# hiroyasuakada/EgoRear

Hardware: AMD Instinct MI355X
Metric: 4-view frames/sec (heatmap+MVFEx+3D lift) (higher is better)
Workload: dtype f32 (fp16x2 split, 22-bit operands, fp32 accumulate)

## Files before the change

### egorear_amd/csrc/egr_conv_chain.hip

```cpp
#include "egr_conv_shared.h"

using namespace egrc;

namespace {

#ifndef CHAIN_SB_G
#define CHAIN_SB_G 1
#endif
#ifndef CHAIN_SB_E
#define CHAIN_SB_E 1
#endif
#define SB_G() do { if (CHAIN_SB_G) __builtin_amdgcn_sched_barrier(0); } while (0)
#define SB_E() do { if (CHAIN_SB_E) __builtin_amdgcn_sched_barrier(0); } while (0)

struct ChainArgs {
    ConvArgs a;
    const void* w2;
    const float* wds2;
    const float* shift1;
    int64_t gw2, gp1;
    int act1;
};

constexpr int OOB = (int)0x80000000;

template <int KS1, int RESK>
__global__ __launch_bounds__(512) void conv_pw_chain_kernel(const ChainArgs ca) {
    constexpr int NCF = 4, KS2 = 8, NPL = 2;
    constexpr bool PIPE = true;
    constexpr int W1B = NCF * KS1 * NPL * 1024, W2B = NCF * KS2 * NPL * 1024;
    constexpr int PR = 16, PATCH = PR * 144;
    constexpr int VEC = 4 * 128 * 4;
    static_assert(W1B + W2B + VEC + 8 * PATCH <= 160 * 1024, "LDS");
    __shared__ __attribute__((aligned(16))) uint8_t lds[W1B + W2B + VEC + 8 * PATCH];
    float* const s_sc1 = reinterpret_cast<float*>(lds + W1B + W2B);
    float* const s_sh1 = s_sc1 + 128;
    float* const s_sc2 = s_sh1 + 128;
    float* const s_sh2 = s_sc2 + 128;
    const ConvArgs& a = ca.a;
    const egr_conv_desc& d = a.d;
    const int grp = blockIdx.z;
    const int tid = threadIdx.x, lane = tid & 63, wave = tid >> 6, p = lane & 31, h = lane >> 5;
    float sa, ads;
    act_prescale(a.amax_in, lane, sa, ads);
    float amx = 0.f;
    unsigned lb0 = lane * 16, lb1 = lane * 16 + 65536;
    asm volatile("" : "+v"(lb0), "+v"(lb1));
    auto wfrag = [&](const int off) __attribute__((always_inline)) {
        return off < 65536 ? *reinterpret_cast<const u32x4*>(lds + lb0 + off) : *reinterpret_cast<const u32x4*>(lds + lb1 + (off - 65536));
    };
    const __amdgpu_buffer_rsrc_t rx = __builtin_amdgcn_make_buffer_rsrc(uniform_ptr(a.x + grp * d.gx), 0, 0x80000000u, 0x00020000);
    const __amdgpu_buffer_rsrc_t ry = __builtin_amdgcn_make_buffer_rsrc(uniform_ptr(a.y + grp * d.gy), 0, 0x80000000u, 0x00020000);
    const __amdgpu_buffer_rsrc_t rr = __builtin_amdgcn_make_buffer_rsrc(uniform_ptr(a.res ? a.res + grp * d.gr : a.x), 0, 0x80000000u, 0x00020000);
    const int HoWo = d.ho * d.wo;
    const int T = (a.M + 31) >> 5, NW = gridDim.x * 8;
    int t = blockIdx.x * 8 + wave;

    auto x_off = [&](int tile) {
        const int m = tile * 32 + p;
        int n, pix;
        if (a.howo_shift >= 0) { n = m >> a.howo_shift; pix = m & (HoWo - 1); }
        else { n = fdiv(m, a.dHoWo); pix = m - n * HoWo; }
        const int xb = a.x_plain ? n * (int)d.xmap.stride_inner : (int)fmap(d.xmap, a.dXin, n);
        return (tile < T && m < a.M) ? (xb + pix * d.ldx) * 4 + h * 16 : OOB;
    };
    u32x4 raw[2 * KS1];
    {
        typedef unsigned u32x2 __attribute__((ext_vector_type(2)));
        auto stage = [&](const uint8_t* img, auto ks_tag, uint8_t* dst0) __attribute__((always_inline)) {
            constexpr int KS = decltype(ks_tag)::value;
            constexpr int NV = NCF * KS * NPL * 64 / 512;
            u32x4 wv[NV];
#pragma unroll
            for (int i = 0; i < NV; ++i) {
                const int v = tid + 512 * i;
                const int cf = v / (KS * 64 * NPL), rem = v - cf * (KS * 64 * NPL);
                wv[i] = *reinterpret_cast<const u32x4*>(img + ((int64_t)cf * (KS / 2) * 2 * NPL) * 1024 + rem * 16);
            }
#pragma unroll
            for (int i = 0; i < NV; ++i) {
                const int v = tid + 512 * i;
                const int lo = v & 63, blk = v >> 6;
                uint8_t* const dst = dst0 + blk * 1024 + (lo & 31) * 16 + (lo >> 5) * 8;
                *reinterpret_cast<u32x2*>(dst) = u32x2{wv[i][0], wv[i][1]};
                *reinterpret_cast<u32x2*>(dst + 512) = u32x2{wv[i][2], wv[i][3]};
            }
        };
        const int xo = x_off(t);
#pragma unroll
        for (int i = 0; i < 2 * KS1; ++i) raw[i] = __builtin_amdgcn_raw_buffer_load_b128(rx, xo + i * 32, 0, 0);
        stage(reinterpret_cast<const uint8_t*>(a.w) + (int64_t)grp * d.gw * 2, std::integral_constant<int, KS1>{}, lds);
        stage(reinterpret_cast<const uint8_t*>(ca.w2) + (int64_t)grp * ca.gw2 * 2, std::integral_constant<int, KS2>{}, lds + W1B);
        if (tid < 128) {
            s_sc1[tid] = ads * a.wds[grp * ca.gp1 + tid];
            s_sh1[tid] = ca.shift1 ? ca.shift1[grp * ca.gp1 + tid] : 0.f;
            s_sc2[tid] = (tid < d.cout) ? ca.wds2[grp * d.gp + tid] * ((a.scale && tid < d.cout) ? a.scale[grp * d.gp + tid] : 1.f) : 1.f;
            s_sh2[tid] = (a.shift && tid < d.cout) ? a.shift[grp * d.gp + tid] : 0.f;
        }
    }
    __syncthreads();

    const float floor1 = (ca.act1 == EGR_ACT_RELU) ? 0.f : -__builtin_inff();
    const float floor_ = (d.act == EGR_ACT_RELU) ? 0.f : -__builtin_inff();
    const bool res_before = d.res_mode == EGR_RES_BEFORE_ACT;
    constexpr int PW[3] = {1, 0, 0}, PX[3] = {0, 1, 0};
    for (; t < T; t += NW) {
#ifdef CHAIN_EXP_NOLOAD
        const int xo_n = OOB;
#else
        const int xo_n = x_off(t + NW);
#endif
        f32x16 acc1[NCF];
// ... 53 lines not shown
                const f32x4 sc = *reinterpret_cast<const f32x4*>(s_sc1 + cf * 32 + 8 * g + 4 * h);
                const f32x4 sh = *reinterpret_cast<const f32x4*>(s_sh1 + cf * 32 + 8 * g + 4 * h);
#pragma unroll
                for (int e = 0; e < 4; ++e) {
                    float v = acc1[cf][4 * g + e] * sc[e] + sh[e];
                    v = v > floor1 ? v : floor1;
                    acc1[cf][4 * g + e] = v;
                    pmax = fmaxf(pmax, fabsf(v));
                }
            }
        pmax = fmaxf(pmax, __shfl_xor(pmax, 32, 64));
        int k2 = 141 - (int)(__float_as_uint(pmax) >> 23);
        k2 = k2 > 60 ? 60 : (k2 < -60 ? -60 : k2);
        const float sa2 = __uint_as_float((unsigned)(127 + k2) << 23), inv2 = __uint_as_float((unsigned)(127 - k2) << 23);
        SB_G();
        f32x16 acc2[NCF];
#pragma unroll
        for (int cf = 0; cf < NCF; ++cf)
#pragma unroll
            for (int r = 0; r < 16; ++r) acc2[cf][r] = 0.f;
        constexpr int S0 = KS1 & 1;
#pragma unroll
        for (int ks = 0; ks < KS2; ++ks) {
            const int cf1 = ks >> 1, g0 = 2 * (ks & 1);
            unsigned xh[4], xl[4];
#pragma unroll
            for (int e = 0; e < 4; ++e) {
                const int r0 = 4 * (g0 + (e >> 1)) + 2 * (e & 1);
                split2_f16(acc1[cf1][r0], acc1[cf1][r0 + 1], sa2, xh[e], xl[e]);
            }
            u32x4 xb[NPL];
            xb[0] = u32x4{xh[0], xh[1], xh[2], xh[3]};
            xb[1] = u32x4{xl[0], xl[1], xl[2], xl[3]};
            if constexpr (PIPE) {
                if (ks + 1 < KS2) read_w2((S0 + ks + 1) & 1, ks + 1);
            } else {
                read_w2(0, ks);
            }
            SB_G();
#pragma unroll
            for (int t3 = 0; t3 < 3; ++t3)
#pragma unroll
                for (int cf = 0; cf < NCF; ++cf)
#ifdef CHAIN_EXP_NOMFMA2
                    if (t3 == 0 && ks == 0)
#endif
                    acc2[cf] = mfma_split<NPL>(wf[PIPE ? ((S0 + ks) & 1) : 0][cf][PW[t3]], xb[PX[t3]], acc2[cf]);
            SB_G();
        }
        SB_G();
#pragma unroll
        for (int i = 0; i < 2 * KS1; ++i) raw[i] = __builtin_amdgcn_raw_buffer_load_b128(rx, xo_n + i * 32, 0, 0);
        SB_G();
        const int m = t * 32 + p;
        int n, pix;
        if (a.howo_shift >= 0) { n = m >> a.howo_shift; pix = m & (HoWo - 1); }
        else { n = fdiv(m, a.dHoWo); pix = m - n * HoWo; }
        const bool live = m < a.M;
        const int yo_p = live ? ((a.y_plain ? n * (int)d.ymap.stride_inner : (int)fmap(d.ymap, a.dYin, n)) + pix * d.ldy) * 4 : OOB;
        int ro_p = OOB, ox_p = 0, oy_p = 0;
        float lx1_p = 0.f, ly1_p = 0.f;
        if constexpr (RESK == 1) {
            if (live) ro_p = ((a.r_plain ? n * (int)d.rmap.stride_inner : (int)fmap(d.rmap, a.dRin, n)) + pix * d.ldr) * 4;
        }
        if constexpr (RESK == 2) {
            const int ho = (a.wo_shift >= 0) ? (pix >> a.wo_shift) : fdiv(pix, a.dWo), wo = pix - ho * d.wo;
            const int hl = d.ho >> 1, wl = d.wo >> 1;
            const float shh = (d.ho > 1) ? (float)(hl - 1) / (float)(d.ho - 1) : 0.f;
            const float sww = (d.wo > 1) ? (float)(wl - 1) / (float)(d.wo - 1) : 0.f;
            const float fy = shh * (float)ho, fx = sww * (float)wo;
            const int y0 = (int)fy, x0 = (int)fx;
            ly1_p = fminf(fmaxf(__builtin_fmaf(shh, (float)ho, -(float)y0), 0.f), 1.f);
            lx1_p = fminf(fmaxf(__builtin_fmaf(sww, (float)wo, -(float)x0), 0.f), 1.f);
            if (live) ro_p = ((a.r_plain ? n * (int)d.rmap.stride_inner : (int)fmap(d.rmap, a.dRin, n)) + (y0 * wl + x0) * d.ldr) * 4;
            ox_p = (x0 + 1 > wl - 1) ? 0 : d.ldr * 4;
            oy_p = (y0 + 1 > hl - 1) ? 0 : wl * d.ldr * 4;
        }
        const int qd = lane & 7, rsub = lane >> 3;
        uint8_t* const patch = lds + W1B + W2B + VEC + wave * PATCH;
        int yo[2][2], ro[2][2], ox[2][2], oy[2][2];
        float lx1[2][2], ly1[2][2];
#pragma unroll
        for (int hp = 0; hp < 2; ++hp)
#pragma unroll
            for (int i = 0; i < 2; ++i) {
                const int src = hp * 16 + i * 8 + rsub;
                yo[hp][i] = __shfl(yo_p, src) + qd * 16;
                if constexpr (RESK != 0) ro[hp][i] = __shfl(ro_p, src) + qd * 16;
                if constexpr (RESK == 2) {
                    ox[hp][i] = __shfl(ox_p, src); oy[hp][i] = __shfl(oy_p, src);
                    lx1[hp][i] = __shfl(lx1_p, src); ly1[hp][i] = __shfl(ly1_p, src);
                }
            }
        constexpr int NR = RESK == 2 ? 4 : (RESK == 1 ? 1 : 0);
        f32x4 rq[2][NR > 0 ? NR : 1];
        auto res_issue = [&](const int st, const int par) __attribute__((always_inline)) {
            if constexpr (RESK != 0) {
                const int hp = st >> 3, cf = (st >> 1) & 3, i = st & 1;
#ifdef CHAIN_EXP_NORES
                if (st > 0) return;
#endif
                const int r0 = (RESK == 1 && cf * 32 + 4 * qd >= d.cout) ? OOB : ro[hp][i] + cf * 128;
                rq[par][0] = __builtin_bit_cast(f32x4, __builtin_amdgcn_raw_buffer_load_b128(rr, r0, 0, 0));
                if constexpr (RESK == 2) {
                    rq[par][1] = __builtin_bit_cast(f32x4, __builtin_amdgcn_raw_buffer_load_b128(rr, ro[hp][i] + ox[hp][i] + cf * 128, 0, 0));
                    rq[par][2] = __builtin_bit_cast(f32x4, __builtin_amdgcn_raw_buffer_load_b128(rr, ro[hp][i] + oy[hp][i] + cf * 128, 0, 0));
                    rq[par][3] = __builtin_bit_cast(f32x4, __builtin_amdgcn_raw_buffer_load_b128(rr, ro[hp][i] + oy[hp][i] + ox[hp][i] + cf * 128, 0, 0));
// ... 307 lines not shown
        const bool live = t < T && m < a.M;
        const int yo_p = live ? ((a.y_plain ? n * (int)d.ymap.stride_inner : (int)fmap(d.ymap, a.dYin, n)) + pix * d.ldy) * 4 : OOB;
        const int qd = lane & 7, rsub = lane >> 3;
        uint8_t* const patch = lds + R * CH + VEC + wave * PATCH;
        int yo[2][2];
#pragma unroll
        for (int hp = 0; hp < 2; ++hp)
#pragma unroll
            for (int i = 0; i < 2; ++i) yo[hp][i] = __shfl(yo_p, hp * 16 + i * 8 + rsub) + qd * 16;
        auto patch_write = [&](const int u) __attribute__((always_inline)) {
            const int hp = u >> 2, cf = u & 3;
            if ((p >> 4) == hp) {
#pragma unroll
                for (int g = 0; g < 4; ++g)
                    *reinterpret_cast<f32x4*>(patch + (p & 15) * 144 + g * 32 + h * 16) =
                        f32x4{acc2[cf][4 * g] * inv2, acc2[cf][4 * g + 1] * inv2, acc2[cf][4 * g + 2] * inv2, acc2[cf][4 * g + 3] * inv2};
            }
        };
        patch_write(0);
#pragma unroll
        for (int u = 0; u < 8; ++u) {
            const int hp = u >> 2, cf = u & 3;
            __builtin_amdgcn_wave_barrier();
            f32x4 vv[2];
#pragma unroll
            for (int i = 0; i < 2; ++i) vv[i] = *reinterpret_cast<const f32x4*>(patch + (i * 8 + rsub) * 144 + qd * 16);
            const int c = cf * 32 + 4 * qd;
            const f32x4 sc = *reinterpret_cast<const f32x4*>(s_sc2 + c), sh = *reinterpret_cast<const f32x4*>(s_sh2 + c);
            const bool cok = c < d.cout;
            asm volatile("s_waitcnt lgkmcnt(0)" ::: "memory");
            __builtin_amdgcn_wave_barrier();
            if (u + 1 < 8) patch_write(u + 1);
#pragma unroll
            for (int i = 0; i < 2; ++i) {
                f32x4 v = vv[i];
#pragma unroll
                for (int e = 0; e < 4; ++e) {
                    float tt = v[e] * sc[e] + sh[e];
                    tt = tt > floor_ ? tt : floor_;
                    v[e] = tt;
                }
                if (cok && yo[hp][i] >= 0) amx = fmaxf(fmaxf(amx, fmaxf(fabsf(v[0]), fabsf(v[1]))), fmaxf(fabsf(v[2]), fabsf(v[3])));
                __builtin_amdgcn_raw_buffer_store_b128(__builtin_bit_cast(u32x4, v), ry, cok ? yo[hp][i] + cf * 128 : OOB, 0, 0);
            }
        }
    }
    if (a.amax_out) amax_flush(a.amax_out, amx, (int)blockIdx.x * NWV + wave);
}

int g_chain_blocks = getenv("EGR_CONV_CHAIN_BLOCKS") ? atoi(getenv("EGR_CONV_CHAIN_BLOCKS")) : 256;

}

extern "C" int egr_conv1x1_chain_f32(const egr_conv_desc* dd, const float* x, const void* w1, const float* shift2, const float* res, float* y,
                                     const egr_conv_aux* aux, const egr_chain_aux* chain, void* stream) {
    if (!dd || !x || !w1 || !y || !aux || !chain || !aux->w_descale || !aux->amax_in || !chain->w2 || !chain->w2_descale) return EGR_ENULL;
    ChainArgs ca;
    ConvArgs& a = ca.a;
    a = ConvArgs{};
    a.d = *dd;
    egr_conv_desc& d = a.d;
    if (d.groups <= 0) d.groups = 1;
    if (d.kh != 1 || d.kw != 1 || d.stride != 1 || d.pad != 0 || d.h != d.ho || d.w != d.wo || d.transposed || d.out_nchw || d.split_k > 1) return EGR_EINVAL;
    const bool big = d.cin == 256 && chain->cmid == 256;
    if (!big && ((d.cin != 64 && d.cin != 128) || chain->cmid != 128)) return EGR_EINVAL;
    if (d.cout <= 0 || d.cout > 128 || d.cout % 4 != 0) return EGR_EINVAL;
    if (big && d.res_mode != EGR_RES_NONE) return EGR_EINVAL;
    if (d.w_format != EGR_W_F16X2 || d.n <= 0 || d.ho <= 0 || d.wo <= 0 || d.groups > 65535) return EGR_EINVAL;
    if ((d.act != EGR_ACT_NONE && d.act != EGR_ACT_RELU) || (chain->act1 != EGR_ACT_NONE && chain->act1 != EGR_ACT_RELU)) return EGR_EINVAL;
    if (d.res_mode != EGR_RES_NONE && !res) return EGR_ENULL;
    if (d.res_mode == EGR_RES_UP2_BEFORE_ACT && ((d.ho | d.wo) & 1)) return EGR_EINVAL;
    if (d.ldx % 4 != 0 || d.ldy % 4 != 0 || (d.res_mode && d.ldr % 4 != 0)) return EGR_EINVAL;
    if (((uintptr_t)x | (uintptr_t)w1 | (uintptr_t)chain->w2 | (uintptr_t)y | (uintptr_t)res) & 15) return EGR_EINVAL;
    if (((uintptr_t)aux->amax_in | (uintptr_t)aux->amax_out) & 3) return EGR_EINVAL;
    if (d.xmap.n_inner <= 0 || d.ymap.n_inner <= 0 || (d.res_mode && d.rmap.n_inner <= 0)) return EGR_EINVAL;
    if (((d.xmap.stride_inner | d.xmap.stride_outer | d.ymap.stride_inner | d.ymap.stride_outer) % 4) != 0) return EGR_EINVAL;
    if (d.res_mode && ((d.rmap.stride_inner | d.rmap.stride_outer) % 4) != 0) return EGR_EINVAL;
    if (d.groups > 1 && (((d.gx | d.gp | d.gy | d.gr | chain->gp1) % 4) != 0 || (d.gw | chain->gw2) % 8 != 0)) return EGR_EINVAL;
    const int64_t M64 = (int64_t)d.n * d.ho * d.wo;
    if (M64 >= (1LL << 31)) return EGR_EINVAL;
    auto span = [](const egr_nmap& m, int n) {
        const int o = (n - 1) / m.n_inner, i = (n - 1 < m.n_inner ? n - 1 : m.n_inner - 1);
        return (int64_t)i * m.stride_inner + (int64_t)o * m.stride_outer;
    };
    if ((span(d.xmap, d.n) + (int64_t)d.h * d.w * d.ldx) * 4 + 64 >= (1LL << 31)) return EGR_EINVAL;
    if ((span(d.ymap, d.n) + (int64_t)d.ho * d.wo * d.ldy) * 4 >= (1LL << 31)) return EGR_EINVAL;
    if (d.res_mode && (span(d.rmap, d.n) + (int64_t)d.ho * d.wo * d.ldr) * 4 >= (1LL << 31)) return EGR_EINVAL;
    a.x = x; a.w = static_cast<const float*>(w1); a.shift = shift2; a.res = res; a.y = y;
    a.wds = aux->w_descale; a.amax_in = aux->amax_in; a.amax_out = aux->amax_out;
    a.M = (int)M64;
    a.Npad = 128;
    a.K = d.cin;
    auto log2_exact = [](int v) { int l = 0; while ((1 << l) < v) ++l; return ((1 << l) == v) ? l : -1; };
    a.howo_shift = log2_exact(d.ho * d.wo);
    a.wo_shift = log2_exact(d.wo);
    a.x_plain = d.xmap.n_inner >= d.n;
    a.y_plain = d.ymap.n_inner >= d.n;
    a.r_plain = d.res_mode ? (d.rmap.n_inner >= d.n) : 1;
    a.dHoWo = make_fastdiv(d.ho * d.wo);
    a.dWo = make_fastdiv(d.wo);
    a.dXin = make_fastdiv(d.xmap.n_inner);
    a.dYin = make_fastdiv(d.ymap.n_inner);
    a.dRin = make_fastdiv(d.res_mode ? d.rmap.n_inner : 1);
    a.cblocks = d.cin / BK;
    a.taps = 1;
    a.ktiles = a.cblocks;
    ca.w2 = chain->w2; ca.wds2 = chain->w2_descale; ca.shift1 = chain->shift1; ca.gw2 = chain->gw2; ca.gp1 = chain->gp1; ca.act1 = chain->act1;
    int nblk = g_chain_blocks / d.groups;
    if (nblk < 1) nblk = 1;
    const int t32 = (a.M + 31) / 32;
    if (nblk * 8 > t32) nblk = (t32 + 7) / 8;
    const dim3 grid((unsigned)nblk, 1, (unsigned)d.groups);
    const int resk = d.res_mode == EGR_RES_NONE ? 0 : (d.res_mode == EGR_RES_UP2_BEFORE_ACT ? 2 : 1);
    hipStream_t s = (hipStream_t)stream;
    if (big) {
        static const int nwv = getenv("EGR_CONV_CHAIN_BIG_WAVES") ? atoi(getenv("EGR_CONV_CHAIN_BIG_WAVES")) : 8;
        if (nwv == 8) {
            hipLaunchKernelGGL((conv_pw2_kernel<0, 8>), grid, dim3(512), 0, s, ca);
        } else {
            int nb4 = 2 * g_chain_blocks / d.groups;
            if (nb4 < 1) nb4 = 1;
            if (nb4 * 4 > t32) nb4 = (t32 + 3) / 4;
            hipLaunchKernelGGL((conv_pw2_kernel<0, 4>), dim3((unsigned)nb4, 1, (unsigned)d.groups), dim3(256), 0, s, ca);
        }
        return egr_launch_status();
    }
    if (d.cin == 64) {
        if (resk == 0) hipLaunchKernelGGL((conv_pw_chain_kernel<4, 0>), grid, dim3(512), 0, s, ca);
        else if (resk == 1) hipLaunchKernelGGL((conv_pw_chain_kernel<4, 1>), grid, dim3(512), 0, s, ca);
        else hipLaunchKernelGGL((conv_pw_chain_kernel<4, 2>), grid, dim3(512), 0, s, ca);
    } else {
        if (resk == 0) hipLaunchKernelGGL((conv_pw_chain_kernel<8, 0>), grid, dim3(512), 0, s, ca);
        else if (resk == 1) hipLaunchKernelGGL((conv_pw_chain_kernel<8, 1>), grid, dim3(512), 0, s, ca);
        else hipLaunchKernelGGL((conv_pw_chain_kernel<8, 2>), grid, dim3(512), 0, s, ca);
    }
    return egr_launch_status();
}
```

### egorear_amd/hip.py

```python
from __future__ import annotations

import ctypes as C
import os
import threading
from typing import Optional, Union

import torch

_HERE = os.path.dirname(os.path.abspath(__file__))
LIB_PATH = os.environ.get("EGR_LIB") or os.path.join(_HERE, "csrc", "libegorear_hip.so")

ACT_NONE, ACT_RELU, ACT_GELU = 0, 1, 2
RES_NONE, RES_BEFORE_ACT, RES_AFTER_ACT, RES_UP2_BEFORE_ACT = 0, 1, 2, 3



import contextlib
import dataclasses
import sys
import types


class _on_default:

    def __init__(self, fn):
        self.fn = fn
        self.__doc__ = fn.__doc__

    def __get__(self, obj, cls):
        return types.MethodType(self.fn, obj if obj is not None else cls())


@dataclasses.dataclass
class LaunchPolicy:
    w_format: str = "f16x2"
    h2: bool = True
    x6_min_rows: int = 4096
    x6_min_flops: float = 5e8
    x6_train_min_rows: int = 8192
    x6_train_min_flops: float = 4e9
    chain: bool = True
    chain_min_rows: int = 8192
    chain_big: bool = True
    chain_big_min_rows: int = 65536
    wgrad_x6: bool = True
    wgrad_force: bool = False
    layer_h2: bool = True
    fused_layer: bool = True
    fused_query: bool = True
    train_one_product: bool = False

    @classmethod
    def from_env(cls, env=None) -> "LaunchPolicy":
        e = os.environ if env is None else env
        fmt = e.get("EGR_W_FORMAT", "f16x2")
        fp16 = fmt in ("f16x2", "f16")
        tfmt = e.get("EGR_TRAIN_FORMAT", "")
        if tfmt not in ("", "f16") or (tfmt == "f16" and fmt != "f16"):
            raise ValueError("egorear_amd: EGR_TRAIN_FORMAT=f16 is the only value, and it requires EGR_W_FORMAT=f16")
        return cls(train_one_product=tfmt == "f16", w_format=fmt, h2=fp16,
                   x6_min_rows=int(e.get("EGR_X6_MIN_ROWS", "4096")), x6_min_flops=float(e.get("EGR_X6_MIN_FLOPS", "5e8")),
                   x6_train_min_rows=int(e.get("EGR_X6_TRAIN_MIN_ROWS", "8192")), x6_train_min_flops=float(e.get("EGR_X6_TRAIN_MIN_FLOPS", "4e9")),
                   chain=e.get("EGR_CONV_CHAIN", "1") != "0", chain_min_rows=int(e.get("EGR_CONV_CHAIN_MIN_ROWS", "8192")),
                   chain_big=e.get("EGR_CONV_CHAIN_BIG", "1") != "0", chain_big_min_rows=int(e.get("EGR_CONV_CHAIN_BIG_MIN_ROWS", "65536")),
                   wgrad_x6=fmt != "f32", layer_h2=fp16 and e.get("EGR_LAYER_H2", "1") != "0",
                   fused_layer=e.get("EGR_FUSED_LAYER", "1") != "0", fused_query=e.get("EGR_FUSED_QUERY", "1") != "0")

    def replace(self, **kw) -> "LaunchPolicy":
        return dataclasses.replace(self, **kw)

    def pack_key(self) -> tuple:
        key = (self.w_format, self.h2, self.layer_h2)
        return key + ("train_f16",) if self.train_one_product else key

    def exact(self) -> "LaunchPolicy":
        return self.replace(w_format="bf16x3", h2=False, layer_h2=False)

    @_on_default
    def fast(self) -> "LaunchPolicy":
        return self.replace(w_format="f16", h2=True, layer_h2=True)

    @_on_default
    def fast_training(self) -> "LaunchPolicy":
        return self.fast().replace(train_one_product=True)

    @property
    def fp16_scheme(self) -> bool:
        return self.w_format in ("f16x2", "f16")


POLICY = LaunchPolicy.from_env()
_POLICY_TLS = threading.local()


def policy() -> LaunchPolicy:
    cur = getattr(_POLICY_TLS, "cur", None)
    return cur if cur is not None else POLICY


@contextlib.contextmanager
def use_policy(p: Optional[LaunchPolicy]):
    if p is None:
        yield
        return
    old = getattr(_POLICY_TLS, "cur", None)
    _POLICY_TLS.cur = p
    try:
        yield
    finally:
        _POLICY_TLS.cur = old


def install_policy_properties(module_name: str, mapping: dict) -> None:
    def make(field):
        return property(lambda self: getattr(policy(), field), lambda self, v: setattr(POLICY, field, v))
    mod = sys.modules[module_name]
    mod.__class__ = type("_PolicyModule", (types.ModuleType,), {name: make(field) for name, field in mapping.items()})


install_policy_properties(__name__, {
    "H2": "h2", "X6_MIN_ROWS": "x6_min_rows", "X6_MIN_FLOPS": "x6_min_flops", "X6_TRAIN_MIN_ROWS": "x6_train_min_rows",
    "X6_TRAIN_MIN_FLOPS": "x6_train_min_flops", "CHAIN": "chain", "CHAIN_MIN_ROWS": "chain_min_rows", "CHAIN_BIG": "chain_big",
    "CHAIN_BIG_MIN_ROWS": "chain_big_min_rows", "WGRAD_X6": "wgrad_x6", "WGRAD_FORCE": "wgrad_force"})

EXPORTS = [
    "egr_conv2d_nhwc_f32", "egr_stem_conv7x7_f32", "egr_maxpool_nhwc_f32", "egr_upsample2x_nhwc_f32",
    "egr_avgpool_nhwc_f32", "egr_argmax_rows_f32", "egr_layernorm_f32", "egr_joint_mha_f32", "egr_msda_gather_f32",
    "egr_fisheye_project_f32", "egr_linear_smallk_f32", "egr_jqa_sum_f32", "egr_tokens_to_nhwc_f32", "egr_version",
    "egr_device_arch", "egr_conv_force_config", "egr_preprocess_u8_f32", "egr_pose_metrics_f32", "egr_gt_heatmap_f32", "egr_conv_debug_stamps", "egr_conv2d_wgrad_f32", "egr_conv2d_masked_f32", "egr_up2_relu_head_f32",
    "egr_msda_fwd_f32", "egr_msda_bwd_f32", "egr_w6_elems", "egr_pack_w6_f32", "egr_pack_w6_many_f32", "egr_joint_layer_f32",
    "egr_preprocess_fused_u8_f32", "egr_preprocess_band_rows", "egr_conv_set_persist", "egr_stem_conv7x7_pool_f32",
    "egr_stem_w6_bytes", "egr_pack_stem_w6_f32", "egr_stem_conv7x7_x6_f32", "egr_wgrad_last_kernel", "egr_conv_last_kernel", "egr_conv_set_tap", "egr_conv_set_tapx", "egr_conv_set_splitk_fused", "egr_fisheye_project2_f32", "egr_pack_layer_w_f32", "egr_pack_layer_wh2_f32",
    "egr_conv2d_nhwc_ex_f32", "egr_wh2_elems", "egr_pack_wh2_f32", "egr_absmax_f32", "egr_stem_conv7x7_x6_ex_f32", "egr_stem_wh2_bytes", "egr_pack_stem_wh2_f32", "egr_stem_conv7x7_h2_f32",
    "egr_pack_wh2_many_f32", "egr_conv2d_masked_ex_f32", "egr_conv2d_wgrad_ex_f32", "egr_wgrad_last_h2", "egr_wgrad_last_planes",
    "egr_wstream_image_bytes", "egr_pack_wstream_f32", "egr_linear_wstream_workspace_bytes", "egr_linear_wstream_f32", "egr_conv1x1_chain_f32",
    "egr_jqa_query_f32", "egr_pose_query_f32", "egr_layer_set_planes", "egr_head_set_persist", "egr_heatmap_metrics_f32",
    "egr_conv_plan", "egr_soft_argmax_f32", "egr_soft_argmax_bwd_f32", "egr_coord_l1_f32",
    "egr_triangulate_f32", "egr_triangulate_bwd_f32", "egr_volume_fuse_f32", "egr_volume_fuse_bwd_f32",
    "egr_peaks_f32", "egr_consensus_f32",
]


class NMap(C.Structure):
    _fields_ = [("n_inner", C.c_int32), ("stride_inner", C.c_int64), ("stride_outer", C.c_int64)]


class ConvDesc(C.Structure):
    _fields_ = [
        ("n", C.c_int32), ("h", C.c_int32), ("w", C.c_int32), ("cin", C.c_int32), ("cout", C.c_int32),
        ("kh", C.c_int32), ("kw", C.c_int32), ("stride", C.c_int32), ("pad", C.c_int32),
        ("ho", C.c_int32), ("wo", C.c_int32), ("ldx", C.c_int32), ("ldy", C.c_int32), ("ldr", C.c_int32),
        ("xmap", NMap), ("ymap", NMap), ("rmap", NMap),
        ("act", C.c_int32), ("res_mode", C.c_int32), ("out_nchw", C.c_int32), ("split_k", C.c_int32),
        ("groups", C.c_int32),
        ("gx", C.c_int64), ("gw", C.c_int64), ("gp", C.c_int64), ("gy", C.c_int64), ("gr", C.c_int64),
        ("grs", C.c_int64), ("grm", C.c_int64),
        ("transposed", C.c_int32), ("w_format", C.c_int32),
    ]


class ConvAux(C.Structure):
    _fields_ = [("w_descale", C.c_void_p), ("amax_in", C.c_void_p), ("amax_out", C.c_void_p),
                ("bn_partials", C.c_void_p), ("bn_tiles_out", C.c_void_p), ("bn_capacity", C.c_int64)]


class ConvPlan(C.Structure):
    _fields_ = [(n, C.c_int32) for n in ("route", "bm", "bn", "variant", "planes", "tiles_m", "tiles_n", "grid_x", "grid_y", "grid_z", "block",
                                         "split_k", "ktiles_per_split", "persistent", "cls_mode", "fused_reduce", "reduce_pass", "bn_slabs")]


ROUTE_F32_TILED, ROUTE_SPLIT_TILED, ROUTE_TAP, ROUTE_TAP2, ROUTE_STREAM_1X1, ROUTE_SMALL_F32, ROUTE_TAPX = range(7)
W_F16X2, W_F16X1, W_F16X1T = 4, 8, 16


class ChainAux(C.Structure):
    _fields_ = [("w2", C.c_void_p), ("w2_descale", C.c_void_p), ("shift1", C.c_void_p), ("cmid", C.c_int32), ("act1", C.c_int32),
                ("gw2", C.c_int64), ("gp1", C.c_int64)]


class LayerDesc(C.Structure):
    _P = C.c_void_p
    _fields_ = ([(n, C.c_int32) for n in ("B", "J", "V", "C", "heads", "cf", "groups", "ffn_dim")] +
                [("eps", C.c_float), ("mha_scale", C.c_float)] +
                [(n, C.c_void_p) for n in ("x", "g", "e", "sigma", "rowmask",
                                           "w_fold", "c_fold", "w_out", "b_out", "w_fuse", "b_fuse", "ln1_g", "ln1_b",
                                           "w_qkv", "b_qkv", "w_mo", "b_mo", "ln2_g", "ln2_b", "w_f0", "b_f0", "w_f1", "b_f1", "ln3_g", "ln3_b",
                                           "x_out", "w_ol", "b_ol", "ol_out")] +
                [("ol_n", C.c_int32), ("w_packed", C.c_int32)] +
                [(n, C.c_void_p) for n in ("lnp_g", "lnp_b", "xn_out", "w_r0", "b_r0", "w_r2", "b_r2", "anchors3d", "pred_out",
                                           "w_h0", "b_h0", "h0_out", "amax_h0")] +
                [("h0_n", C.c_int32)])


class JqaQueryDesc(C.Structure):
    _fields_ = ([(n, C.c_int32) for n in ("B", "J", "C", "groups", "kb", "pool_hw", "ol_n", "w_packed")] +
                [(n, C.c_void_p) for n in ("t", "s32", "w_hp2", "b_hp2", "w_bfb", "b_bfb", "embed", "w_q", "b_q", "w_ol", "b_ol",
                                           "x_out", "ol_out")])


class PoseQueryDesc(C.Structure):
    _fields_ = ([(n, C.c_int32) for n in ("B", "J", "C", "ol_n", "w_packed")] +
                [(n, C.c_void_p) for n in ("h1", "w_m2", "b_m2", "ctm", "cams", "w_qg0", "b_qg0", "w_qg2", "b_qg2", "w_qg4", "b_qg4",
                                           "w_ol", "b_ol", "pred_out", "anchors3d_out", "anchors2d_out", "valid_out", "x_out", "ol_out")])


def _load() -> C.CDLL:
    if not os.path.exists(LIB_PATH):
        raise ImportError(
            f"{LIB_PATH} not found: build it with `python -m egorear_amd.csrc.build` "
            "(or __graft_entry__.build()).  egorear_amd has no CPU / PyTorch fallback.")
    lib = C.CDLL(LIB_PATH)
    vp, i32, i64, f32 = C.c_void_p, C.c_int32, C.c_int64, C.c_float
    lib.egr_conv2d_nhwc_f32.argtypes = [C.POINTER(ConvDesc), vp, vp, vp, vp, vp, vp, vp, vp, vp, C.c_size_t, vp]
    lib.egr_conv2d_nhwc_ex_f32.argtypes = [C.POINTER(ConvDesc), vp, vp, vp, vp, vp, vp, vp, vp, vp, C.c_size_t, C.POINTER(ConvAux), vp]
    lib.egr_conv_plan.argtypes = [C.POINTER(ConvDesc), vp, vp, vp, vp, vp, vp, vp, vp, vp, vp, C.c_size_t, C.POINTER(ConvAux), C.POINTER(ConvPlan)]
    lib.egr_conv1x1_chain_f32.argtypes = [C.POINTER(ConvDesc), vp, vp, vp, vp, vp, C.POINTER(ConvAux), C.POINTER(ChainAux), vp]
    lib.egr_fill_f32.argtypes = [vp, f32, i64, vp]
    lib.egr_fill_f32.restype = C.c_int
    lib.egr_absmax_f32.argtypes = [vp, i64, vp, vp]
    lib.egr_wh2_elems.restype = C.c_int64
    lib.egr_wh2_elems.argtypes = [i32, i32]
    lib.egr_pack_wh2_f32.argtypes = [vp, i32, i32, i32, vp, vp, vp]
    lib.egr_stem_conv7x7_f32.argtypes = [vp, NMap, i32, i32, i32, vp, vp, vp, vp, i32, i64, vp]
    lib.egr_stem_conv7x7_pool_f32.argtypes = [vp, NMap, i32, i32, i32, vp, vp, vp, vp, i32, i64, vp]
    lib.egr_wgrad_last_kernel.argtypes = []
    lib.egr_wgrad_last_planes.argtypes = []
    lib.egr_conv_last_kernel.argtypes = []
    lib.egr_conv_set_tap.argtypes = [i32]
    lib.egr_conv_set_tapx.argtypes = [i32, i32, i32]
    lib.egr_conv_set_splitk_fused.argtypes = [i32]
    lib.egr_stem_w6_bytes.restype = C.c_int64
    lib.egr_stem_w6_bytes.argtypes = []
    lib.egr_pack_stem_w6_f32.argtypes = [vp, i32, vp, vp]
    lib.egr_stem_conv7x7_x6_f32.argtypes = [vp, NMap, i32, i32, i32, vp, vp, vp, vp, i32, i32, i64, vp]
    lib.egr_stem_conv7x7_x6_ex_f32.argtypes = [vp, NMap, i32, i32, i32, vp, vp, vp, vp, i32, i32, i64, vp, vp]
    lib.egr_stem_wh2_bytes.restype = C.c_int64
    lib.egr_stem_wh2_bytes.argtypes = []
    lib.egr_pack_stem_wh2_f32.argtypes = [vp, i32, vp, vp, vp]
    lib.egr_stem_conv7x7_h2_f32.argtypes = [vp, NMap, i32, i32, i32, vp, vp, vp, vp, vp, i32, i32, i64, vp, vp]
    lib.egr_wstream_image_bytes.restype = C.c_int64
    lib.egr_wstream_image_bytes.argtypes = [i32, i32]
    lib.egr_pack_wstream_f32.argtypes = [vp, i32, i32, vp, vp, vp]
    lib.egr_linear_wstream_workspace_bytes.restype = C.c_int64
    lib.egr_linear_wstream_workspace_bytes.argtypes = [i32, i32, i32]
    lib.egr_linear_wstream_f32.argtypes = [vp, i64, i32, i32, vp, vp, vp, i32, i32, vp, vp, i64, vp, vp, i64, vp]
    lib.egr_maxpool_nhwc_f32.argtypes = [vp, vp, i32, i32, i32, i32, i32, i32, i32, vp]
    lib.egr_upsample2x_nhwc_f32.argtypes = [vp, i32, vp, i32, i32, i32, i32, i32, i32, vp]
    lib.egr_avgpool_nhwc_f32.argtypes = [vp, vp, i32, i32, i32, vp]
    lib.egr_argmax_rows_f32.argtypes = [vp, i32, i32, i32, f32, vp, vp, vp, vp, vp]
    lib.egr_soft_argmax_f32.argtypes = [vp, i32, i32, i32, f32, i32, i32, f32, vp, vp, vp, vp, vp, vp, vp]
    lib.egr_soft_argmax_bwd_f32.argtypes = [vp, vp, vp, vp, vp, vp, i32, i32, i32, f32, i32, i32, i32, vp, vp]
    lib.egr_triangulate_f32.argtypes = [vp, vp, vp, vp, i32, i32, i32, f32, f32, f32, f32, vp, vp, vp, vp, vp]
    lib.egr_triangulate_bwd_f32.argtypes = [vp, vp, vp, vp, i32, i32, i32, f32, f32, f32, f32, vp, vp, vp, vp, vp]
    lib.egr_volume_fuse_f32.argtypes = [vp, vp, vp, vp, vp, vp, i32, i32, i32, i32, i32, i32, f32, f32, f32, vp, vp, vp, vp, vp, vp]
    lib.egr_volume_fuse_bwd_f32.argtypes = [vp, vp, vp, vp, vp, vp, i32, i32, i32, i32, i32, i32, f32, f32, f32, vp, vp, vp, vp]
    lib.egr_peaks_f32.argtypes = [vp, i32, i32, i32, i32, i32, i32, f32, f32, vp, vp, vp, vp, vp]
    lib.egr_consensus_f32.argtypes = [vp, vp, vp, vp, vp, i32, i32, i32, i32, f32, f32, f32, i32, f32, vp, vp, vp, vp, vp, vp, vp]
    lib.egr_coord_l1_f32.argtypes = [vp, vp, vp, i32, i32, f32, vp, vp, vp]
    lib.egr_layernorm_f32.argtypes = [vp, vp, vp, vp, vp, i32, i32, f32, i32, vp]
    lib.egr_joint_mha_f32.argtypes = [vp, vp, i32, i32, i32, i32, f32, vp]
    lib.egr_msda_gather_f32.argtypes = [vp, i32, vp, i32, vp, vp, vp, i32, i32, i32, i32, i32, i32, vp, vp, vp, vp, i32, vp]
    lib.egr_fisheye_project_f32.argtypes = [vp, vp, vp, i32, i32, vp, vp, vp, vp]
    lib.egr_fisheye_project2_f32.argtypes = [vp, vp, vp, vp, i32, i32, vp, vp, vp, vp]
    lib.egr_linear_smallk_f32.argtypes = [vp, i64, i64, vp, vp, vp, i32, i32, i32, i32, i32, vp]
    lib.egr_jqa_sum_f32.argtypes = [vp, vp, vp, vp, i32, i32, i32, i32, vp]
    lib.egr_tokens_to_nhwc_f32.argtypes = [vp, vp, i32, i32, i32, vp]
    lib.egr_version.restype = C.c_char_p
    lib.egr_w6_elems.restype = C.c_int64
    lib.egr_device_arch.argtypes = [C.c_char_p, i32]
# ... 495 lines not shown
        return False
    return x.n * x.h * x.w >= (pol.chain_big_min_rows if big else pol.chain_min_rows)


def conv1x1_chain(x: Img, w1, w2, cmid: int, cout: int, *, shift1=None, shift2=None, act1: int = ACT_RELU, act2: int = ACT_NONE,
                  res: Optional[Img] = None, res_mode: int = RES_NONE, out: Optional[Img] = None, groups: int = 1,
                  amax_out: Optional[torch.Tensor] = None) -> Img:
    if not chain_eligible(x, w1, w2, cmid, cout, groups, res_mode=res_mode):
        raise LaunchError("egr_conv1x1_chain_f32", EINVAL)
    ng = x.n // groups
    gx = ng * x.nstride if groups > 1 else 0
    xg = Img(x.t[:ng], amax=x.amax) if groups > 1 else x
    for w in (w1, w2):
        if not w.h2_used:
            if w.f32 is not None:
                pack_wh2_into(w)
            w.h2_used = True
    d = ConvDesc()
    d.w_format = 4
    d.n, d.h, d.w, d.cin, d.cout = xg.n, xg.h, xg.w, xg.c, cout
    d.kh, d.kw, d.stride, d.pad, d.ho, d.wo = 1, 1, 1, 0, xg.h, xg.w
    d.ldx, d.xmap = xg.ld, xg.nmap()
    d.act, d.res_mode, d.split_k, d.transposed, d.out_nchw = act2, res_mode, 1, 0, 0
    full = out
    if out is None:
        full = Img(torch.empty((x.n, x.h, x.w, cout), device=x.t.device, dtype=torch.float32))
        out = full
    if out.n != x.n or (out.h, out.w, out.c) != (x.h, x.w, cout):
        raise RuntimeError("egorear_amd.conv1x1_chain: output shape does not match")
    gy = ng * out.nstride if groups > 1 else 0
    og = Img(out.t[:ng]) if groups > 1 else out
    d.ldy, d.ymap = og.ld, og.nmap()
    gr = 0
    if res_mode != RES_NONE:
        if res is None or res.n != x.n:
            raise RuntimeError("egorear_amd.conv1x1_chain: res_mode set without a residual of groups x n images")
        if res_mode == RES_UP2_BEFORE_ACT and (2 * res.h != x.h or 2 * res.w != x.w or res.c < cout):
            raise RuntimeError("egorear_amd.conv1x1_chain: the upsampled residual must be exactly half the output resolution")
        gr = ng * res.nstride if groups > 1 else 0
        rg = Img(res.t[:ng]) if groups > 1 else res
        d.ldr, d.rmap = rg.ld, rg.nmap()
    else:
        d.rmap = NMap(1, 0, 0)
    d.groups, d.gx, d.gw, d.gp, d.gy, d.gr = groups, gx, (w1.h2_gstride if groups > 1 else 0), (128 if groups > 1 else 0), gy, gr
    for t, nm, need, gs in ((shift1, "shift1", cmid, w1.npad), (shift2, "shift2", cout, 128)):
        if t is not None and t.numel() < ((groups - 1) * gs + need):
            raise RuntimeError(f"egorear_amd.conv1x1_chain: {nm} shorter than expected")
    if amax_out is not None and (amax_out.numel() != 64 or amax_out.dtype != torch.int32 or not amax_out.is_contiguous()):
        raise RuntimeError("egorear_amd.conv1x1_chain: amax_out must be 64 contiguous int32 slots")
    aux = ConvAux(_p(w1.h2_ds).value, _p(x.amax, torch.int32).value, _p(amax_out, torch.int32).value if amax_out is not None else None, None, None, 0)
    ch = ChainAux(_p(w2.h2, torch.float16).value, _p(w2.h2_ds).value, _p(shift1).value if shift1 is not None else None, cmid, act1,
                  (w2.h2_gstride if groups > 1 else 0), (w1.npad if groups > 1 else 0))
    M = ng * x.h * x.w
    _launch("egr_conv1x1_chain_f32", lib.egr_conv1x1_chain_f32, C.byref(d), _p(xg.t), _p(w1.h2, torch.float16), _p(shift2),
            _p(res.t) if res is not None else None, _p(og.t), C.byref(aux), C.byref(ch), _stream(),
            flops=2.0 * M * groups * (cmid * x.c + cout * cmid), nbytes=4.0 * groups * (M * (cout + x.c) + cmid * x.c + cout * cmid),
            tag=f"h2 chain G{groups} M{M} N{cout} K{x.c} k1s1 cin{x.c} mid{cmid}" if PROFILE is not None else "")
    full.tag(amax_out)
    return full


def wgrad_records(x: Img, dy: Img, amax_arena: Optional["AmaxArena"]) -> None:
    if not policy().h2 or amax_arena is None:
        return
    for im in (x, dy):
        if im.amax is None and im.t.is_contiguous():
            rec = amax_arena.new()
            if rec is not None:
                absmax_record(im.t, rec)
                im.amax = rec


def conv2d_wgrad(x: Img, dy: Img, kh: int, kw: int, stride: int, pad: int, workspace: torch.Tensor, *, want_bias: bool = False,
                 dw: Optional[torch.Tensor] = None, db: Optional[torch.Tensor] = None, accumulate: bool = False, groups: int = 1,
                 x6: Optional[bool] = None, amax_arena: Optional["AmaxArena"] = None, gx: Optional[int] = None, gy: Optional[int] = None,
                 one_product: Optional[bool] = None):
    cin, cout = x.c, dy.c
    interleaved = gx is not None or gy is not None
    if interleaved and (gx is None or gy is None):
        raise RuntimeError("egorear_amd.conv2d_wgrad: gx and gy go together")
    if dy.n != x.n or (not interleaved and x.n % groups):
        raise RuntimeError("egorear_amd.conv2d_wgrad: image counts do not match / not divisible by groups")
    ng = x.n if interleaved else x.n // groups
    if ((x.h + 2 * pad - kh) // stride + 1, (x.w + 2 * pad - kw) // stride + 1) != (dy.h, dy.w):
        raise RuntimeError("egorear_amd.conv2d_wgrad: dy does not match the forward output geometry")
    d = ConvDesc()
    d.n, d.h, d.w, d.cin, d.cout = ng, x.h, x.w, cin, cout
    d.kh, d.kw, d.stride, d.pad, d.ho, d.wo = kh, kw, stride, pad, dy.h, dy.w
    d.ldx, d.ldy, d.rmap = x.ld, dy.ld, NMap(1, 0, 0)
    d.xmap, d.ymap = NMap(ng, x.nstride, 0), NMap(ng, dy.nstride, 0)
    K = kh * kw * cin
    d.groups, d.gx, d.gy, d.gw, d.gp = groups, (gx if interleaved else ng * x.nstride), (gy if interleaved else ng * dy.nstride), cout * K, cout
    if x6 is None and policy().wgrad_force and policy().wgrad_x6:
        x6 = "force"
    d.w_format = 3 if x6 == "force" else (1 if (policy().wgrad_x6 if x6 is None else x6) else 0)
    M = ng * dy.h * dy.w
    split = d.w_format == 3 or (d.w_format == 1 and M >= 1024 and 2.0 * M * cout * K * groups >= 4e9)
    if split:
        wgrad_records(x, dy, amax_arena)
    h2 = split and policy().h2 and x.amax is not None and dy.amax is not None
    h1 = h2 and (policy().train_one_product if one_product is None else bool(one_product))
    if h2:
        d.w_format |= W_F16X2 | (W_F16X1 if h1 else 0)
    shape_w, shape_b = ((groups, cout, K), (groups, cout)) if groups > 1 else ((cout, K), (cout,))
    if dw is None:
        dw = torch.empty(shape_w, device=x.t.device, dtype=torch.float32)
    elif dw.numel() != groups * cout * K:
        raise RuntimeError("egorear_amd.conv2d_wgrad: dw has the wrong size")
# ... 783 lines not shown
```

### include/egorear_hip.h

```cpp
#ifndef EGOREAR_HIP_H
#define EGOREAR_HIP_H

#include <stddef.h>
#include <stdint.h>

#ifdef __cplusplus
extern "C" {
#endif

#define EGR_EINVAL (-1)
#define EGR_ENULL (-2)
#define EGR_EWORKSPACE (-3)

enum { EGR_ACT_NONE = 0, EGR_ACT_RELU = 1, EGR_ACT_GELU = 2 };
enum { EGR_RES_NONE = 0, EGR_RES_BEFORE_ACT = 1, EGR_RES_AFTER_ACT = 2,
       EGR_RES_UP2_BEFORE_ACT = 3  };

typedef struct {
    int32_t n_inner;
    int64_t stride_inner;
    int64_t stride_outer;
} egr_nmap;

typedef struct {
// ... 17 lines not shown
       EGR_W_F16X2 = 4 ,
       EGR_W_F16X1 = 8,
       EGR_W_F16X1T = 16 };

int64_t egr_w6_elems(int32_t npad, int32_t k);
int egr_pack_w6_f32(const float* w, int32_t npad, int32_t k, int32_t groups, void* img, void* stream);

typedef struct {
    const float* w;
    void* img;
    int32_t npad, k, groups, reserved;
    int64_t first_block;
} egr_w6_job;
int egr_pack_w6_many_f32(const egr_w6_job* jobs, int32_t count, int64_t total_blocks, void* stream);

int64_t egr_wh2_elems(int32_t npad, int32_t k);
int egr_pack_wh2_f32(const float* w, int32_t npad, int32_t k, int32_t groups, void* img, float* descale, void* stream);
typedef struct {
    const float* w;
    void* img;
    float* descale;
    int32_t npad, k, groups, reserved;
    int64_t first_rblock, first_pblock;
} egr_wh2_job;
int egr_pack_wh2_many_f32(const egr_wh2_job* jobs, int32_t count, int64_t total_rblocks, int64_t total_pblocks, void* stream);

int egr_conv2d_nhwc_f32(const egr_conv_desc* d, const float* x, const float* w,
                        const float* scale , const float* shift ,
                        const float* res , const float* rowscale ,
                        const uint8_t* rowmask ,
                        float* y, float* workspace, size_t workspace_floats, void* stream);

typedef struct {
    const float* w_descale;
    const uint32_t* amax_in;
    uint32_t* amax_out;
    double* bn_partials;
    int32_t* bn_tiles_out;
    int64_t bn_capacity;
} egr_conv_aux;
int egr_conv2d_nhwc_ex_f32(const egr_conv_desc* d, const float* x, const void* w, const float* scale, const float* shift,
                           const float* res, const float* rowscale, const uint8_t* rowmask, float* y, float* workspace,
                           size_t workspace_floats, const egr_conv_aux* aux , void* stream);

typedef struct {
    const void* w2;
    const float* w2_descale;
    const float* shift1;
    int32_t cmid, act1;
    int64_t gw2, gp1;
} egr_chain_aux;
int egr_conv1x1_chain_f32(const egr_conv_desc* d, const float* x, const void* w1, const float* shift2, const float* res, float* y,
                          const egr_conv_aux* aux, const egr_chain_aux* chain, void* stream);

int egr_conv2d_masked_f32(const egr_conv_desc* d, const float* x, const float* w, const float* res, const float* mask, float* y,
                          float* workspace, size_t workspace_floats, void* stream);
int egr_conv2d_masked_ex_f32(const egr_conv_desc* d, const float* x, const void* w, const float* res, const float* mask, float* y,
                             float* workspace, size_t workspace_floats, const egr_conv_aux* aux, void* stream);

typedef enum {
    EGR_ROUTE_F32_TILED = 0,
    EGR_ROUTE_SPLIT_TILED = 1,
    EGR_ROUTE_TAP = 2,
    EGR_ROUTE_TAP2 = 3,
    EGR_ROUTE_STREAM_1X1 = 4,
    EGR_ROUTE_SMALL_F32 = 5,
    EGR_ROUTE_TAPX = 6
} egr_conv_route;
typedef struct {
    int32_t route;
    int32_t bm, bn;
    int32_t variant;
    int32_t planes;
    int32_t tiles_m, tiles_n;
    int32_t grid_x, grid_y, grid_z, block;
    int32_t split_k, ktiles_per_split;
    int32_t persistent;
    int32_t cls_mode;
    int32_t fused_reduce;
    int32_t reduce_pass;
    int32_t bn_slabs;
} egr_conv_plan_t;
int egr_conv_plan(const egr_conv_desc* d, const float* x, const void* w, const float* scale, const float* shift,
                  const float* res, const float* rowscale, const uint8_t* rowmask, const float* mask, const float* y,
                  const float* workspace, size_t workspace_floats, const egr_conv_aux* aux, egr_conv_plan_t* out);

int egr_conv2d_wgrad_f32(const egr_conv_desc* d, const float* x, const float* dy, float* dw, float* db,
                         float* workspace, size_t workspace_floats, int32_t accumulate, void* stream);
int egr_conv2d_wgrad_ex_f32(const egr_conv_desc* d, const float* x, const float* dy, float* dw, float* db, float* workspace,
                            size_t workspace_floats, int32_t accumulate, const uint32_t* amax_x, const uint32_t* amax_dy, void* stream);
int egr_wgrad_last_h2(void);
int egr_wgrad_last_planes(void);
int egr_wgrad_last_kernel(void);

int egr_conv_force_config(int cfg);
int egr_conv_last_kernel(void);
int egr_conv_set_splitk_fused(int on);
int egr_conv_set_tap(int on);
int egr_conv_set_tapx(int32_t on, int32_t min_tiles, int32_t blocks);
int egr_conv_set_persist(int slots, int max_ktiles);

int egr_up2_relu_head_f32(const float* lo, int32_t n, int32_t h, int32_t w, int32_t cin, const float* wgt, const float* bias,
                          int32_t cout, float* planes, int32_t n_inner, int64_t stride_inner, int64_t stride_outer,
                          int32_t groups, int64_t gy, void* stream);
int egr_head_set_persist(int on);

// ... 196 lines not shown
```

Baseline: 6897.

## Use 2x16 pixel tiles and XCD-aware block remap in upsampled-residual chain

For the 1x1 conv chain with the 2x-upsampled residual, each 32-row tile now covers two image rows by 16 columns instead of 32 consecutive pixels. This lets the bilinear residual reads share low-resolution source rows within a wave. Block indices are also permuted so that consecutive tiles land on the same XCD, which should improve L2 locality. The cost is extra index arithmetic, and the path only applies when the width is a power of two of at least 32.

```diff
diff --git a/egorear_amd/csrc/egr_conv_chain.hip b/egorear_amd/csrc/egr_conv_chain.hip
--- a/egorear_amd/csrc/egr_conv_chain.hip
+++ b/egorear_amd/csrc/egr_conv_chain.hip
@@ -20,12 +20,14 @@
     const float* shift1;
     int64_t gw2, gp1;
     int act1;
+    int t2d_shift, xcd_q;
 };
 
 constexpr int OOB = (int)0x80000000;
 
-template <int KS1, int RESK>
+template <int KS1, int RESK, bool LOC = false>
 __global__ __launch_bounds__(512) void conv_pw_chain_kernel(const ChainArgs ca) {
+    static_assert(!LOC || RESK == 2, "the local variant is about the up-sampled residual");
     constexpr int NCF = 4, KS2 = 8, NPL = 2;
     constexpr bool PIPE = true;
     constexpr int W1B = NCF * KS1 * NPL * 1024, W2B = NCF * KS2 * NPL * 1024;
@@ -54,10 +56,18 @@
     const __amdgpu_buffer_rsrc_t rr = __builtin_amdgcn_make_buffer_rsrc(uniform_ptr(a.res ? a.res + grp * d.gr : a.x), 0, 0x80000000u, 0x00020000);
     const int HoWo = d.ho * d.wo;
     const int T = (a.M + 31) >> 5, NW = gridDim.x * 8;
-    int t = blockIdx.x * 8 + wave;
+    const int bx = (LOC && ca.xcd_q > 0) ? ((int)blockIdx.x & 7) * ca.xcd_q + ((int)blockIdx.x >> 3) : (int)blockIdx.x;
+    auto m_of = [&](int tile) {
+        if (LOC && ca.t2d_shift >= 0) {
+            const int rp = tile >> ca.t2d_shift, c = tile - (rp << ca.t2d_shift);
+            return ((2 * rp + (p >> 4)) << a.wo_shift) + c * 16 + (p & 15);
+        }
+        return tile * 32 + p;
+    };
+    int t = bx * 8 + wave;
 
     auto x_off = [&](int tile) {
-        const int m = tile * 32 + p;
+        const int m = m_of(tile);
         int n, pix;
         if (a.howo_shift >= 0) { n = m >> a.howo_shift; pix = m & (HoWo - 1); }
         else { n = fdiv(m, a.dHoWo); pix = m - n * HoWo; }
@@ -217,7 +227,7 @@
 #pragma unroll
         for (int i = 0; i < 2 * KS1; ++i) raw[i] = __builtin_amdgcn_raw_buffer_load_b128(rx, xo_n + i * 32, 0, 0);
         SB_G();
-        const int m = t * 32 + p;
+        const int m = m_of(t);
         int n, pix;
         if (a.howo_shift >= 0) { n = m >> a.howo_shift; pix = m & (HoWo - 1); }
         else { n = fdiv(m, a.dHoWo); pix = m - n * HoWo; }
@@ -631,8 +641,8 @@
 
 }
 
-extern "C" int egr_conv1x1_chain_f32(const egr_conv_desc* dd, const float* x, const void* w1, const float* shift2, const float* res, float* y,
-                                     const egr_conv_aux* aux, const egr_chain_aux* chain, void* stream) {
+extern "C" int egr_conv1x1_chain_ex_f32(const egr_conv_desc* dd, const float* x, const void* w1, const float* shift2, const float* res, float* y,
+                                        const egr_conv_aux* aux, const egr_chain_aux* chain, int flags, void* stream) {
     if (!dd || !x || !w1 || !y || !aux || !chain || !aux->w_descale || !aux->amax_in || !chain->w2 || !chain->w2_descale) return EGR_ENULL;
     ChainArgs ca;
     ConvArgs& a = ca.a;
@@ -691,6 +701,13 @@
     if (nblk * 8 > t32) nblk = (t32 + 7) / 8;
     const dim3 grid((unsigned)nblk, 1, (unsigned)d.groups);
     const int resk = d.res_mode == EGR_RES_NONE ? 0 : (d.res_mode == EGR_RES_UP2_BEFORE_ACT ? 2 : 1);
+    ca.t2d_shift = -1;
+    ca.xcd_q = 0;
+    const bool loc = (flags & EGR_CHAIN_LOCAL) && resk == 2 && a.wo_shift >= 5;
+    if (loc) {
+        ca.t2d_shift = a.wo_shift - 4;
+        if (nblk % 8 == 0) ca.xcd_q = nblk / 8;
+    }
     hipStream_t s = (hipStream_t)stream;
     if (big) {
         static const int nwv = getenv("EGR_CONV_CHAIN_BIG_WAVES") ? atoi(getenv("EGR_CONV_CHAIN_BIG_WAVES")) : 8;
@@ -707,11 +724,18 @@
     if (d.cin == 64) {
         if (resk == 0) hipLaunchKernelGGL((conv_pw_chain_kernel<4, 0>), grid, dim3(512), 0, s, ca);
         else if (resk == 1) hipLaunchKernelGGL((conv_pw_chain_kernel<4, 1>), grid, dim3(512), 0, s, ca);
+        else if (loc) hipLaunchKernelGGL((conv_pw_chain_kernel<4, 2, true>), grid, dim3(512), 0, s, ca);
         else hipLaunchKernelGGL((conv_pw_chain_kernel<4, 2>), grid, dim3(512), 0, s, ca);
     } else {
         if (resk == 0) hipLaunchKernelGGL((conv_pw_chain_kernel<8, 0>), grid, dim3(512), 0, s, ca);
         else if (resk == 1) hipLaunchKernelGGL((conv_pw_chain_kernel<8, 1>), grid, dim3(512), 0, s, ca);
+        else if (loc) hipLaunchKernelGGL((conv_pw_chain_kernel<8, 2, true>), grid, dim3(512), 0, s, ca);
         else hipLaunchKernelGGL((conv_pw_chain_kernel<8, 2>), grid, dim3(512), 0, s, ca);
     }
     return egr_launch_status();
 }
+
+extern "C" int egr_conv1x1_chain_f32(const egr_conv_desc* dd, const float* x, const void* w1, const float* shift2, const float* res, float* y,
+                                     const egr_conv_aux* aux, const egr_chain_aux* chain, void* stream) {
+    return egr_conv1x1_chain_ex_f32(dd, x, w1, shift2, res, y, aux, chain, EGR_CHAIN_LOCAL, stream);
+}
diff --git a/egorear_amd/hip.py b/egorear_amd/hip.py
--- a/egorear_amd/hip.py
+++ b/egorear_amd/hip.py
@@ -43,6 +43,7 @@
     chain_min_rows: int = 8192
     chain_big: bool = True
     chain_big_min_rows: int = 65536
+    chain_local: bool = True
     wgrad_x6: bool = True
     wgrad_force: bool = False
     layer_h2: bool = True
@@ -63,6 +64,7 @@
                    x6_train_min_rows=int(e.get("EGR_X6_TRAIN_MIN_ROWS", "8192")), x6_train_min_flops=float(e.get("EGR_X6_TRAIN_MIN_FLOPS", "4e9")),
                    chain=e.get("EGR_CONV_CHAIN", "1") != "0", chain_min_rows=int(e.get("EGR_CONV_CHAIN_MIN_ROWS", "8192")),
                    chain_big=e.get("EGR_CONV_CHAIN_BIG", "1") != "0", chain_big_min_rows=int(e.get("EGR_CONV_CHAIN_BIG_MIN_ROWS", "65536")),
+                   chain_local=e.get("EGR_CONV_CHAIN_LOCAL", "1") != "0",
                    wgrad_x6=fmt != "f32", layer_h2=fp16 and e.get("EGR_LAYER_H2", "1") != "0",
                    fused_layer=e.get("EGR_FUSED_LAYER", "1") != "0", fused_query=e.get("EGR_FUSED_QUERY", "1") != "0")
 
@@ -121,7 +123,7 @@
 install_policy_properties(__name__, {
     "H2": "h2", "X6_MIN_ROWS": "x6_min_rows", "X6_MIN_FLOPS": "x6_min_flops", "X6_TRAIN_MIN_ROWS": "x6_train_min_rows",
     "X6_TRAIN_MIN_FLOPS": "x6_train_min_flops", "CHAIN": "chain", "CHAIN_MIN_ROWS": "chain_min_rows", "CHAIN_BIG": "chain_big",
-    "CHAIN_BIG_MIN_ROWS": "chain_big_min_rows", "WGRAD_X6": "wgrad_x6", "WGRAD_FORCE": "wgrad_force"})
+    "CHAIN_BIG_MIN_ROWS": "chain_big_min_rows", "CHAIN_LOCAL": "chain_local", "WGRAD_X6": "wgrad_x6", "WGRAD_FORCE": "wgrad_force"})
 
 EXPORTS = [
     "egr_conv2d_nhwc_f32", "egr_stem_conv7x7_f32", "egr_maxpool_nhwc_f32", "egr_upsample2x_nhwc_f32",
@@ -133,7 +135,7 @@
     "egr_stem_w6_bytes", "egr_pack_stem_w6_f32", "egr_stem_conv7x7_x6_f32", "egr_wgrad_last_kernel", "egr_conv_last_kernel", "egr_conv_set_tap", "egr_conv_set_tapx", "egr_conv_set_splitk_fused", "egr_fisheye_project2_f32", "egr_pack_layer_w_f32", "egr_pack_layer_wh2_f32",
     "egr_conv2d_nhwc_ex_f32", "egr_wh2_elems", "egr_pack_wh2_f32", "egr_absmax_f32", "egr_stem_conv7x7_x6_ex_f32", "egr_stem_wh2_bytes", "egr_pack_stem_wh2_f32", "egr_stem_conv7x7_h2_f32",
     "egr_pack_wh2_many_f32", "egr_conv2d_masked_ex_f32", "egr_conv2d_wgrad_ex_f32", "egr_wgrad_last_h2", "egr_wgrad_last_planes",
-    "egr_wstream_image_bytes", "egr_pack_wstream_f32", "egr_linear_wstream_workspace_bytes", "egr_linear_wstream_f32", "egr_conv1x1_chain_f32",
+    "egr_wstream_image_bytes", "egr_pack_wstream_f32", "egr_linear_wstream_workspace_bytes", "egr_linear_wstream_f32", "egr_conv1x1_chain_f32", "egr_conv1x1_chain_ex_f32",
     "egr_jqa_query_f32", "egr_pose_query_f32", "egr_layer_set_planes", "egr_head_set_persist", "egr_heatmap_metrics_f32",
     "egr_conv_plan", "egr_soft_argmax_f32", "egr_soft_argmax_bwd_f32", "egr_coord_l1_f32",
     "egr_triangulate_f32", "egr_triangulate_bwd_f32", "egr_volume_fuse_f32", "egr_volume_fuse_bwd_f32",
@@ -171,6 +173,7 @@
 
 ROUTE_F32_TILED, ROUTE_SPLIT_TILED, ROUTE_TAP, ROUTE_TAP2, ROUTE_STREAM_1X1, ROUTE_SMALL_F32, ROUTE_TAPX = range(7)
 W_F16X2, W_F16X1, W_F16X1T = 4, 8, 16
+CHAIN_LOCAL_BIT = 1
 
 
 class ChainAux(C.Structure):
@@ -215,6 +218,7 @@
     lib.egr_conv2d_nhwc_ex_f32.argtypes = [C.POINTER(ConvDesc), vp, vp, vp, vp, vp, vp, vp, vp, vp, C.c_size_t, C.POINTER(ConvAux), vp]
     lib.egr_conv_plan.argtypes = [C.POINTER(ConvDesc), vp, vp, vp, vp, vp, vp, vp, vp, vp, vp, C.c_size_t, C.POINTER(ConvAux), C.POINTER(ConvPlan)]
     lib.egr_conv1x1_chain_f32.argtypes = [C.POINTER(ConvDesc), vp, vp, vp, vp, vp, C.POINTER(ConvAux), C.POINTER(ChainAux), vp]
+    lib.egr_conv1x1_chain_ex_f32.argtypes = [C.POINTER(ConvDesc), vp, vp, vp, vp, vp, C.POINTER(ConvAux), C.POINTER(ChainAux), C.c_int, vp]
     lib.egr_fill_f32.argtypes = [vp, f32, i64, vp]
     lib.egr_fill_f32.restype = C.c_int
     lib.egr_absmax_f32.argtypes = [vp, i64, vp, vp]
@@ -816,8 +820,8 @@
     ch = ChainAux(_p(w2.h2, torch.float16).value, _p(w2.h2_ds).value, _p(shift1).value if shift1 is not None else None, cmid, act1,
                   (w2.h2_gstride if groups > 1 else 0), (w1.npad if groups > 1 else 0))
     M = ng * x.h * x.w
-    _launch("egr_conv1x1_chain_f32", lib.egr_conv1x1_chain_f32, C.byref(d), _p(xg.t), _p(w1.h2, torch.float16), _p(shift2),
-            _p(res.t) if res is not None else None, _p(og.t), C.byref(aux), C.byref(ch), _stream(),
+    _launch("egr_conv1x1_chain_f32", lib.egr_conv1x1_chain_ex_f32, C.byref(d), _p(xg.t), _p(w1.h2, torch.float16), _p(shift2),
+            _p(res.t) if res is not None else None, _p(og.t), C.byref(aux), C.byref(ch), CHAIN_LOCAL_BIT if policy().chain_local else 0, _stream(),
             flops=2.0 * M * groups * (cmid * x.c + cout * cmid), nbytes=4.0 * groups * (M * (cout + x.c) + cmid * x.c + cout * cmid),
             tag=f"h2 chain G{groups} M{M} N{cout} K{x.c} k1s1 cin{x.c} mid{cmid}" if PROFILE is not None else "")
     full.tag(amax_out)
diff --git a/include/egorear_hip.h b/include/egorear_hip.h
--- a/include/egorear_hip.h
+++ b/include/egorear_hip.h
@@ -93,6 +93,9 @@
 } egr_chain_aux;
 int egr_conv1x1_chain_f32(const egr_conv_desc* d, const float* x, const void* w1, const float* shift2, const float* res, float* y,
                           const egr_conv_aux* aux, const egr_chain_aux* chain, void* stream);
+#define EGR_CHAIN_LOCAL 1
+int egr_conv1x1_chain_ex_f32(const egr_conv_desc* d, const float* x, const void* w1, const float* shift2, const float* res, float* y,
+                             const egr_conv_aux* aux, const egr_chain_aux* chain, int flags, void* stream);
 
 int egr_conv2d_masked_f32(const egr_conv_desc* d, const float* x, const float* w, const float* res, const float* mask, float* y,
                           float* workspace, size_t workspace_floats, void* stream);
```

After: 6884. About the same (-0.2%).
